# jasonyaw/CDAE

Hardware: AMD Instinct MI355X
Metric: users/sec (whole node) K=200 ML-10M-shape; Recall@10 parity (higher is better)
Workload: dtype f32

## Files before the change

cdae_amd/csrc/cdae_hip.hip:

```cpp
#include <hip/hip_runtime.h>

#include <cstring>

#include <rocprim/rocprim.hpp>

#include <algorithm>
#include <atomic>
#include <condition_variable>
#include <deque>
#include <mutex>
#include <thread>
#include <chrono>
#include <cmath>
#include <cstdarg>
#include <cstdlib>
#include <cstdio>
#include <cstring>
#include <numeric>
#include <string>
#include <vector>

#include "../../include/cdae_hip.h"
#include "cdae_internal.hpp"
#include "cdae_kernels.hpp"
// ... 1364 lines not shown
  place(CDAE_P_B, h->Kp); place(CDAE_P_B_AG, h->Kp);
  h->n_shared = o;
  CHK(dev_alloc(&h->d_shared, h->n_shared));
  HIPCHK(hipMemset(h->d_shared, 0, h->n_shared * sizeof(float)));
  const size_t WR = (size_t)h->wu_rows();
  h->cnt[CDAE_P_WU] = h->cnt[CDAE_P_WU_AG] = WR * h->Kp;
  CHK(dev_alloc(&h->d_Wu, WR * h->Kp));
  CHK(dev_alloc(&h->d_Wu_ag, WR * h->Kp));
  HIPCHK(hipMemset(h->d_Wu, 0, std::max<size_t>(WR * h->Kp, 1) * sizeof(float)));
  HIPCHK(hipMemset(h->d_Wu_ag, 0, std::max<size_t>(WR * h->Kp, 1) * sizeof(float)));
  if (h->cfg.linear_function) {
    h->cnt[CDAE_P_UU] = h->cnt[CDAE_P_UU_AG] = WR * h->Kp;
    CHK(dev_alloc(&h->d_Uu, WR * h->Kp));
    CHK(dev_alloc(&h->d_Uu_ag, WR * h->Kp));
  }

  const uint32_t B = (uint32_t)std::min<uint64_t>(h->B, U);
  uint64_t emax = 0;
  for (uint64_t s0 = 0; s0 < U; ++s0) {
    const uint64_t s1 = std::min<uint64_t>(U, s0 + B);
    emax = std::max<uint64_t>(emax, (uint64_t)(row_ptr[s1] - row_ptr[s0]));
  }
  h->ex_per_pos = h->mf == 2 ? 2u * h->hp.num_neg : 1u + h->hp.num_neg;
  h->Ecap = emax * h->ex_per_pos;
  h->h_grow_ptr.clear(); h->h_gunit_ptr.clear();
  if (h->shard_sampled()) {
    const int64_t* grp = h->g_row_ptr_src;
    const uint32_t* gcl = h->g_col_src;
    h->g_row_ptr_src = nullptr; h->g_col_src = nullptr;
    if (grp[0] != 0) return fail("whole-row row_ptr[0] must be 0");
    h->h_grow_ptr.assign(grp, grp + U + 1);
    uint64_t gmax = 0;
    for (uint64_t s0 = 0; s0 < U; ++s0) gmax = std::max<uint64_t>(gmax, (uint64_t)(grp[std::min<uint64_t>(U, s0 + B)] - grp[s0]));
    h->Ecap = gmax * h->ex_per_pos;
    const size_t gnnz = (size_t)grp[U];
    CHK(dev_alloc(&h->d_grow_ptr, U + 1)); CHK(dev_alloc(&h->d_gcol, gnnz));
    HIPCHK(hipMemcpy(h->d_grow_ptr, grp, (U + 1) * sizeof(int64_t), hipMemcpyHostToDevice));
    HIPCHK(hipMemcpy(h->d_gcol, gcl, gnnz * sizeof(uint32_t), hipMemcpyHostToDevice));
    h->h_gunit_ptr.assign(U + 1, 0u);
    for (uint64_t u = 0; u < U; ++u)
      h->h_gunit_ptr[u + 1] = h->h_gunit_ptr[u] + (uint32_t)((grp[u + 1] - grp[u] + h->hp.unit_pos - 1) / h->hp.unit_pos);
    CHK(dev_alloc(&h->d_gunit_ptr, U + 1));
    HIPCHK(hipMemcpy(h->d_gunit_ptr, h->h_gunit_ptr.data(), (U + 1) * sizeof(uint32_t), hipMemcpyHostToDevice));
    std::vector<uint32_t> guser(h->h_gunit_ptr[U]);
    for (uint64_t u = 0; u < U; ++u)
      for (uint32_t g = h->h_gunit_ptr[u]; g < h->h_gunit_ptr[u + 1]; ++g) guser[g] = (uint32_t)u;
    CHK(dev_alloc(&h->d_gunit_user, std::max<size_t>(guser.size(), 1)));
    HIPCHK(hipMemcpy(h->d_gunit_user, guser.data(), guser.size() * sizeof(uint32_t), hipMemcpyHostToDevice));
  }
  h->seq = 0; h->pre_n = 0;
  h->counting_sort = I <= cdae::TILE_SORT_MAX_ITEMS && DEV_ENV("CDAE_SORT_TILE") != nullptr;
  h->bucket_sort = false; h->bucket_ranges = 0; h->cell_units = 0;
  {
    const uint64_t BUCKET_MAX_EXAMPLES = h->cfg.full_output ? 100000 : 600000;
    const uint64_t keys = I + (h->shard_sampled() ? 1u : 0u);
    if (keys <= 65536 && !h->counting_sort && !h->mf_seq && h->Ecap <= BUCKET_MAX_EXAMPLES && h->Ecap > 0 && !DEV_ENV("CDAE_SORT_LIBRARY")) {
      const double b_share = (double)B / (double)U;
      const double draw_items = (double)(h->shard_sampled() ? h->I_global : I);
      const double whole_nnz = h->shard_sampled() ? (double)h->h_grow_ptr[U] : (double)nnz;
      const uint32_t negs = h->mf == 2 ? 2u * h->hp.num_neg - 0u : h->hp.num_neg;
      const double neg_per_item = b_share * whole_nnz * (double)negs / draw_items;
      std::vector<double> wgt(I);
      double total = 0.0;
      for (uint64_t i = 0; i < I; ++i) { wgt[i] = b_share * (double)pop[i] + neg_per_item; total += wgt[i]; }
      const double per_range = std::max(total / 256.0, std::min(2730.0, total / 8.0));
      std::vector<uint32_t> cut{0u};
      double acc = 0.0;
      for (uint64_t i = 0; i < I; ++i) {
        acc += wgt[i];
        if (i + 1 < I && (acc >= per_range || (i + 1) - cut.back() == cdae::BK_ITEMS)) { cut.push_back((uint32_t)(i + 1)); acc = 0.0; }
      }
      cut.push_back((uint32_t)I);
      if (cut.size() - 1 <= cdae::BK_MAX_RANGES) {
        h->bucket_sort = true;
        h->bucket_ranges = (uint32_t)cut.size() - 1;
        CHK(dev_alloc(&h->d_bucket_cut, cut.size()));
        HIPCHK(hipMemcpy(h->d_bucket_cut, cut.data(), cut.size() * sizeof(uint32_t), hipMemcpyHostToDevice));
        if (!h->mf && h->bucket_ranges <= cdae::BKC_MAX_RANGES && h->Ecap < (1ull << (32 - cdae::BKC_ITEM_BITS)) && !DEV_ENV("CDAE_SORT_SCAN")) {
          std::vector<uint16_t> rof(I);
          for (uint32_t r = 0; r + 1 < cut.size(); ++r)
            for (uint32_t i = cut[r]; i < cut[r + 1]; ++i) rof[i] = (uint16_t)r;
          CHK(dev_alloc(&h->d_range_of, (size_t)I));
          HIPCHK(hipMemcpy(h->d_range_of, rof.data(), I * sizeof(uint16_t), hipMemcpyHostToDevice));
        }
      }
    }
  }
  h->h_unit_ptr.assign(U + 1, 0u);
  for (uint64_t u = 0; u < U; ++u)
    h->h_unit_ptr[u + 1] = h->h_unit_ptr[u] + (uint32_t)((row_ptr[u + 1] - row_ptr[u] + h->hp.unit_pos - 1) / h->hp.unit_pos);
  h->unit_cap = 0;
  for (uint64_t s0 = 0; s0 < U; ++s0) {
    const uint64_t s1 = std::min<uint64_t>(U, s0 + B);
    h->unit_cap = std::max(h->unit_cap, h->h_unit_ptr[s1] - h->h_unit_ptr[s0]);
  }
  {
    std::vector<uint32_t> per(U);
    for (uint64_t u = 0; u < U; ++u) per[u] = h->h_unit_ptr[u + 1] - h->h_unit_ptr[u];
    std::partial_sort(per.begin(), per.begin() + B, per.end(), std::greater<uint32_t>());
    uint64_t top = 0;
    for (uint32_t i = 0; i < B; ++i) top += per[i];
    h->unit_cap = (uint32_t)std::max<uint64_t>(h->unit_cap, top);
  }
  if (h->shard_sampled())
    for (uint64_t s0 = 0; s0 < U; ++s0)
      h->unit_cap = std::max(h->unit_cap, h->h_gunit_ptr[std::min<uint64_t>(U, s0 + B)] - h->h_gunit_ptr[s0]);
  CHK(dev_alloc(&h->d_unit_ptr, U + 1));
// ... 1428 lines not shown
```

cdae_amd/csrc/cdae_kernels.hpp:

```cpp
#pragma once
#include <type_traits>

#include <hip/hip_runtime.h>
#include <stdint.h>

#include "../../include/cdae_rng.h"
#include "cdae_exchange_algebra.h"

namespace cdae {

constexpr int WAVE = 64;
constexpr uint32_t SLOT_MASK = 0x0FFFFFFFu;
constexpr uint32_t DUP_PREV_BIT = 1u << 28;
constexpr uint32_t DUP_NEXT_BIT = 1u << 29;
constexpr uint32_t DUP_NONE = 0xFFFFFFFFu;
constexpr uint32_t DUP_STRIPES = 64;
constexpr uint32_t TARGET_BIT = 1u << 30;
constexpr uint32_t INPUT_BIT = 1u << 31;

constexpr uint32_t LATE_MAX = 64;
struct DecodeLate {
  float* Ghot;
  uint32_t* hotdup;
  uint32_t late_rows;
// ... 134 lines not shown

__device__ __forceinline__ float loss_grad(uint32_t loss_type, float pred, float truth) {
  if (loss_type == 0u) return -2.f * (truth - pred);
  return fast_rcp(1.f + fast_exp(-pred)) - truth;
}
__device__ __forceinline__ float loss_eval(uint32_t loss_type, float pred, float truth) {
  if (loss_type == 0u) { float e = truth - pred; return e * e; }
  float ret = (1.f - truth) * pred;
  if (pred > 18.f) return ret + fast_exp(-pred);
  if (pred < -18.f) return ret - pred;
  return ret + log1pf(fast_exp(-pred));
}
__device__ __forceinline__ float activate(const HyperParams& hp, float x) {
  if (hp.linear) return x;
  if (!hp.tanh_act) return x > 18.f ? 1.f : (x < -18.f ? 0.f : fast_rcp(1.f + fast_exp(-x)));
  if (x > 9.f) return 1.f;
  if (x < -9.f) return -1.f;
  float r = fast_exp(-2.f * x);
  return (1.f - r) * fast_rcp(1.f + r);
}
__device__ __forceinline__ float act_deriv(const HyperParams& hp, float z) {
  return hp.linear ? 1.f : (hp.tanh_act ? 1.f - z * z : z - z * z);
}
template <bool ADA>
__device__ __forceinline__ void ada_step_t(const HyperParams& hp, float& p, float& acc, float grad) {
  if (ADA) {
    acc = fmaf(grad, grad, acc);
    p = fmaf(-hp.lr * grad, fast_rcp(fast_sqrt(acc) + hp.beta), p);
  } else {
    p = fmaf(-hp.lr, grad, p);
  }
}
__device__ __forceinline__ void ada_step(const HyperParams& hp, float& p, float& acc, float grad) {
  if (hp.adagrad) ada_step_t<true>(hp, p, acc, grad); else ada_step_t<false>(hp, p, acc, grad);
}

template <int CTRL, int ROW_MASK = 0xF>
__device__ __forceinline__ float dpp_add(float v) {
  const int moved = __builtin_amdgcn_update_dpp(0, __builtin_bit_cast(int, v), CTRL, ROW_MASK, 0xF,  true);
  return v + __builtin_bit_cast(float, moved);
}
__device__ __forceinline__ float wave_sum(float v) {
  v = dpp_add<0xB1>(v);
  v = dpp_add<0x4E>(v);
  v = dpp_add<0x141>(v);
  v = dpp_add<0x140>(v);
  v = dpp_add<0x142>(v);
  v = dpp_add<0x143>(v);
  return __builtin_bit_cast(float, __builtin_amdgcn_readlane(__builtin_bit_cast(int, v), 63));
}

constexpr uint32_t BKC_SLOTS = 32, BKC_ITEM_BITS = 12, BKC_ITEM_MASK = (1u << BKC_ITEM_BITS) - 1u;
constexpr uint32_t BKC_MAX_RANGES = 256;
constexpr uint32_t UNIT_POS_MAX = 128;

struct UnitRef { uint32_t slot, p0, p1; };

__device__ __forceinline__ UnitRef locate_unit(const uint32_t unit_pos, const uint32_t* __restrict__ uptr, uint32_t nb, uint32_t g,
                                               const uint32_t* __restrict__ unit_user = nullptr, uint64_t u0 = 0) {
  uint32_t lo = 0, hi = nb;
  if (unit_user) {
    lo = unit_user[g] - (uint32_t)u0;
  } else {
    while (hi - lo > 1) {
      const uint32_t mid = (lo + hi) >> 1;
      if (uptr[mid] <= g) lo = mid; else hi = mid;
    }
  }
  UnitRef r;
  r.slot = lo;
  r.p0 = (g - uptr[lo]) * unit_pos;
  r.p1 = r.p0 + unit_pos;
  return r;
}

__device__ __forceinline__ int lds_row_contains(const uint32_t* row, uint32_t n, uint32_t item) {
  uint32_t lo = 0, hi = n;
  while (lo < hi) {
    const uint32_t mid = (lo + hi) >> 1;
    if (row[mid] < item) lo = mid + 1; else hi = mid;
  }
  return lo < n && row[lo] == item;
}
constexpr uint32_t SAMPLE_LDS_ROW = 2048;

__global__ void __launch_bounds__(256)
sample_kernel(HyperParams hp, const int64_t* __restrict__ row_ptr, const uint32_t* __restrict__ col,
              const uint32_t* __restrict__ uptr, uint32_t n_units, uint64_t u0, uint32_t nb, uint32_t cidx,
              uint64_t seed, uint32_t epoch, uint32_t* __restrict__ ex_item, uint64_t* __restrict__ ex_val,
              uint16_t* __restrict__ ex_key16 ,
              uint32_t* __restrict__ seg , uint32_t seg_words,
              uint32_t* __restrict__ dup_count, uint32_t* __restrict__ dup_of_ex,
              const uint32_t* __restrict__ unit_user ,
              uint32_t* __restrict__ wg_state ,
              const uint32_t* __restrict__ gpos ,
              uint32_t shard_item0 = 0, uint32_t shard_items = 0, uint32_t draw_items = 0,
              const uint16_t* __restrict__ range_of = nullptr, const uint32_t* __restrict__ range_cut = nullptr, uint32_t n_ranges = 0,
              uint32_t* __restrict__ cells = nullptr, uint32_t* __restrict__ cell_flag = nullptr, uint32_t cell_tag = 0) {
#ifdef CDAE_PREP_SETPRIO
  __builtin_amdgcn_s_setprio(CDAE_PREP_SETPRIO);
#endif
  __shared__ uint32_t lds_rows[4][SAMPLE_LDS_ROW];
  __shared__ uint32_t cell_cnt[4][BKC_MAX_RANGES];
  __shared__ uint32_t cell_lo[BKC_MAX_RANGES];
  if (cells) {
    for (uint32_t i = threadIdx.x; i < n_ranges; i += blockDim.x) cell_lo[i] = range_cut[i];
// ... 1153 lines not shown
      if (dup) { const uint32_t k = len + (uint32_t)__popcll(dmask & below); lrow[k] = cur.di[h2] | DUP_ROW; lg[k] = 1.f; }
      if (mine) { const uint32_t k = len + n_d + (uint32_t)__popcll(mask & below); lrow[k] = cur.item[h2]; lg[k] = cur.g[h2]; }
      len += n_d + n_r;
    }
    __builtin_amdgcn_fence(__ATOMIC_RELEASE, "wavefront");
    __builtin_amdgcn_wave_barrier();
    const bool last = c0 + 2 * WAVE >= n_ex;
    while (len - head >= (uint32_t)TRIP) trip((uint32_t)TRIP);
    if (last || len + 4u * WAVE > GCAP) {
      if (len > head) trip(len - head);
      head = 0; len = 0;
      __builtin_amdgcn_wave_barrier();
    }
    cur = nxt;
  }
  if (lo >= hp.K) {
#pragma unroll
    for (int i = 0; i < NI; ++i) acc[i] = 0.f;
  }
  vstore<NI>(ga.HGpart + ((size_t)part * ga.n_units + unit) * hp.Kp + lo, acc);
  trace_end(hp, 5, unit * 8u + part, t0, n_ex);
}

template <int NI>
__global__ void __launch_bounds__(256)
hidden_gather_kernel(HyperParams hp, const int64_t* __restrict__ row_ptr, const uint32_t* __restrict__ uptr,
                     uint32_t n_units, uint64_t u0, uint32_t nb, const uint32_t* __restrict__ ex_item,
                     const float* __restrict__ G, const float* __restrict__ D0,
                     float* __restrict__ HGpart ,
                     uint32_t explicit_examples ,
                     const uint32_t* __restrict__ dup_of_ex, const float* __restrict__ dup_corr,
                     const uint32_t* __restrict__ unit_user,
                     const uint32_t* __restrict__ late_bits = nullptr ,
                     uint32_t late_words = 0) {
  __shared__ uint32_t gl_row[4][GATHER_CAP];
  __shared__ float gl_g[4][GATHER_CAP];
  __shared__ uint32_t lbits[LATE_BITS_WORDS];
  stage_late_bits(lbits, late_bits, late_words);
  const uint32_t part = blockIdx.x & 7u;
  const uint32_t unit = (blockIdx.x >> 3) * (blockDim.x / WAVE) + threadIdx.x / WAVE;
  if (unit >= n_units) return;
  const GatherArgs ga{row_ptr, uptr, n_units, u0, nb, ex_item, G, D0, HGpart, explicit_examples, dup_of_ex, dup_corr, unit_user,
                      late_bits, late_words, nullptr};
  hidden_gather_role<NI, false>(hp, ga, part, unit, gl_row[threadIdx.x / WAVE], gl_g[threadIdx.x / WAVE], late_bits ? lbits : nullptr);
}

struct FusedGeom {
  uint32_t hot_wgs;
  uint32_t decode_wgs;
  const uint32_t* cold_map;
};
constexpr uint32_t FUSED_LDS_WORDS = 4u * 2u * GATHER_CAP + LATE_BITS_WORDS;
static_assert(4u * ROWS16_LDS_WORDS <= FUSED_LDS_WORDS, "row roles' LDS");
static_assert(3u * (FUSED_LDS_WORDS + 8u) * 4u + 90376u <= 160u * 1024u, "three workgroups of this launch + one of bucket_sort_kernel per CU");
#ifndef CDAE_FUSED_WAVES_PER_SIMD
#define CDAE_FUSED_WAVES_PER_SIMD 3
#endif
template <int NV, int NT, int LOSS, bool ADAGRAD>
__global__ void __launch_bounds__(256, CDAE_FUSED_WAVES_PER_SIMD)
decode_gather_kernel(HyperParams hp, uint32_t hot_rows, FusedGeom geo, DecodeLate late, GatherArgs ga, CDAE_DECODE_PARAMS) {
  constexpr int CH = NT == 0 ? NV : NV + 1;
  constexpr int NI = CH <= 1 ? 1 : (CH <= 2 ? 2 : 4);
  __shared__ uint32_t fused_lds[FUSED_LDS_WORDS + 8u];
  const uint32_t wg = blockIdx.x;
  const uint32_t wid = __builtin_amdgcn_readfirstlane(threadIdx.x / WAVE);
  if (wg < geo.hot_wgs) {
    const uint32_t row = wg * 4u + wid;
    if (row < hot_rows && !CDAE_SKIP_ROLE(hp, 4u)) {
      const unsigned long long t0 = trace_begin(hp);
      __builtin_amdgcn_s_setprio(CDAE_HOT_PRIO);
      decode_row64<NI, LOSS, ADAGRAD, false, true>(hp, row, reinterpret_cast<float*>(fused_lds + wid * ROWS16_LDS_WORDS), ROW64_PARK_WORDS, late,
                                                   CDAE_DECODE_PASS);
      __builtin_amdgcn_s_setprio(0);
      trace_end(hp, 3, row, t0, hp.trace ? hw_place() : 0u);
    }
  } else if (wg < geo.decode_wgs) {
    if (CDAE_SKIP_ROLE(hp, 8u)) return;
    uint32_t* const claim = fused_lds + FUSED_LDS_WORDS;
    if (threadIdx.x < 4) claim[threadIdx.x] = 0u;
    __syncthreads();
    const uint32_t simd = (__builtin_amdgcn_s_getreg((1 << 11) | (4 << 6) | 4) ) & 3u;
    if (threadIdx.x % WAVE == 0) atomicCAS(&claim[simd], 0u, 1u + wid);
    __syncthreads();
    const uint32_t cs[4] = {claim[0], claim[1], claim[2], claim[3]};
    int mine = -1;
#pragma unroll
    for (int q = 0; q < 4; ++q) if (cs[q] == 1u + wid) mine = q;
    if (mine < 0) {
      uint32_t before = 0, cnt = 0;
#pragma unroll
      for (int q = 0; q < 4; ++q) if (cs[q] && cs[q] - 1u < wid) ++before;
      const uint32_t j = wid - before;
#pragma unroll
      for (int q = 0; q < 4; ++q) if (!cs[q]) { if (cnt == j) mine = q; ++cnt; }
    }
    const uint32_t g = geo.cold_map[wg * 4u + (uint32_t)mine];
    if (g == 0xFFFFFFFFu) return;
    const unsigned long long t0 = trace_begin(hp);
    decode_rows16<NV, NT, LOSS, ADAGRAD, true>(hp, hot_rows + g * 4u, fused_lds + wid * ROWS16_LDS_WORDS, CDAE_DECODE_PASS);
    trace_end(hp, 4, hot_rows / 4u + g, t0, hp.trace ? hw_place() : 0u);
  } else {
    uint32_t* const lbits = fused_lds + 4u * 2u * GATHER_CAP;
    stage_late_bits(lbits, ga.late_bits, ga.late_words);
    const uint32_t gw = wg - geo.decode_wgs;
    const uint32_t part = gw & 7u, unit = (gw >> 3) * 4u + wid;
    if (unit >= ga.n_units) return;
    hidden_gather_role<NI, true>(hp, ga, part, unit, fused_lds + wid * 2u * GATHER_CAP,
// ... 718 lines not shown
```

cdae_amd/csrc/cdae_sort_kernels.hpp:

```cpp
#pragma once
#include <hip/hip_runtime.h>
#include <stdint.h>

#include "cdae_kernels.hpp"

namespace cdae {

#ifndef CDAE_SEGSORT_THREADS
#define CDAE_SEGSORT_THREADS 256
#endif
constexpr uint32_t SEGSORT_THREADS = CDAE_SEGSORT_THREADS;
#ifndef CDAE_SEGSORT_ITEMS
#define CDAE_SEGSORT_ITEMS 8
#endif
constexpr uint32_t SEGSORT_ITEMS = CDAE_SEGSORT_ITEMS;
#ifndef CDAE_SEGSORT_WINDOW
#define CDAE_SEGSORT_WINDOW 3072
#endif
constexpr uint32_t SEGSORT_WINDOW = CDAE_SEGSORT_WINDOW;

constexpr uint32_t TILE_SORT_MAX_ITEMS = 32768;
#ifndef CDAE_TILE_EX
#define CDAE_TILE_EX 4096
#endif
// ... 141 lines not shown
      uint32_t rank = 0;
      if (in_lds) {
        const uint64_t v = raw[q];
        uint32_t r[8] = {0, 0, 0, 0, 0, 0, 0, 0};
        uint32_t j = a;
        for (; j + 8 <= b; j += 8) {
#pragma unroll
          for (int t = 0; t < 8; ++t) r[t] += raw[j + t] < v ? 1u : 0u;
        }
        for (; j < b; ++j) r[0] += raw[j] < v ? 1u : 0u;
        rank = ((r[0] + r[1]) + (r[2] + r[3])) + ((r[4] + r[5]) + (r[6] + r[7]));
        srt[a + rank] = v;
      } else {
        const uint64_t v = bucketed_val[p0 + q];
        for (uint32_t j = a; j < b; ++j) rank += bucketed_val[p0 + j] < v ? 1u : 0u;
        sorted_val[p0 + a + rank] = v;
      }
    }
    __syncthreads();
    uint32_t my_dups = 0;
    for (uint32_t q = threadIdx.x; q < n; q += blockDim.x) {
      const uint32_t k = item_of(k0, p0 + q);
      const uint32_t a = item_off[k] - p0, b = item_off[k + 1] - p0;
      uint64_t v = in_lds ? srt[q] : sorted_val[p0 + q];
      const uint32_t slot = (uint32_t)v & SLOT_MASK;
      uint32_t flags = 0;
      if (q > a && ((uint32_t)(in_lds ? srt[q - 1] : sorted_val[p0 + q - 1]) & SLOT_MASK) == slot) flags |= DUP_PREV_BIT;
      if (q + 1 < b && ((uint32_t)(in_lds ? srt[q + 1] : sorted_val[p0 + q + 1]) & SLOT_MASK) == slot) flags |= DUP_NEXT_BIT;
      if (in_lds || flags) sorted_val[p0 + q] = v | flags;
      if (flags & DUP_PREV_BIT) ++my_dups;
    }
    uint32_t off = my_dups ? atomicAdd(&blk_count, my_dups) : 0u;
    __syncthreads();
    if (threadIdx.x == 0) { blk_base = blk_count ? atomicAdd(dup_count + blockIdx.x % stripes, blk_count) : 0u; blk_count = 0u; }
    __syncthreads();
    if (my_dups) {
      off += blk_base;
      const uint32_t stripe_cap = dup_cap / stripes, stripe0 = (blockIdx.x % stripes) * stripe_cap;
      for (uint32_t q = threadIdx.x; q < n; q += blockDim.x) {
        const uint64_t v = sorted_val[p0 + q];
        if (!((uint32_t)v & DUP_PREV_BIT)) continue;
        const uint32_t idx = off < stripe_cap ? stripe0 + off : DUP_NONE;
        ++off;
        dup_of_pos[p0 + q] = idx;
        dup_of_ex[(uint32_t)(v >> 32)] = idx;
      }
    }
    __syncthreads();
    k0 = k1;
  }
}

constexpr uint32_t BK_THREADS = 512;
constexpr uint32_t BK_WINDOW = 4096;
constexpr uint32_t BK_ITEMS = 2048;
constexpr uint32_t BK_WAVE_LIST = BK_WINDOW / (BK_THREADS / 64);
constexpr uint32_t BK_SPIN_CAP = 1u << 21;
constexpr uint32_t BK_MAX_RANGES = 1024;
constexpr uint32_t BK_CELL_UNITS_MAX = 16384;
constexpr size_t BK_LDS_BYTES = (size_t)BK_WINDOW * 8 * 2 + (size_t)BK_WINDOW * 2 + (size_t)(BK_ITEMS + 1) * 4 * 2 + 64 * 4;
static_assert(BK_ITEMS <= 4 * BK_THREADS && BK_ITEMS <= (1u << BKC_ITEM_BITS), "bk_block_scan takes 4 counters per thread; a cell entry holds the item in BKC_ITEM_BITS bits");

__device__ __forceinline__ void bk_block_scan(uint32_t* v, uint32_t n, uint32_t* wave_tot) {
  const uint32_t t = threadIdx.x, lane = t % WAVE, wid = t / WAVE;
  uint32_t c[4], sum = 0;
#pragma unroll
  for (uint32_t j = 0; j < 4; ++j) { c[j] = 4u * t + j < n ? v[4u * t + j] : 0u; sum += c[j]; }
  uint32_t incl = sum;
#pragma unroll
  for (int off = 1; off < WAVE; off <<= 1) {
    const uint32_t o = __shfl_up(incl, off, WAVE);
    if ((int)lane >= off) incl += o;
  }
  if (lane == WAVE - 1) wave_tot[wid] = incl;
  __syncthreads();
  uint32_t before = 0;
  for (uint32_t w = 0; w < wid; ++w) before += wave_tot[w];
  uint32_t run = before + incl - sum;
#pragma unroll
  for (uint32_t j = 0; j < 4; ++j) { if (4u * t + j < n) v[4u * t + j] = run; run += c[j]; }
  if (t == BK_THREADS - 1) v[n] = run;
  __syncthreads();
}

constexpr uint32_t BK_UNROLL = 4;
template <typename F>
__device__ __forceinline__ void bk_scan_keys(const uint16_t* __restrict__ keys, uint32_t n_ex, F&& f) {
  const uint32_t n8 = n_ex & ~7u;
  constexpr uint32_t ROUND = BK_THREADS * 8u * BK_UNROLL;
  uint4 q[BK_UNROLL], nx[BK_UNROLL];
  auto request = [&](uint4 (&dst)[BK_UNROLL], uint32_t r0) {
#pragma unroll
    for (uint32_t u = 0; u < BK_UNROLL; ++u) {
      const uint32_t e0 = r0 + (u * BK_THREADS + threadIdx.x) * 8u;
      dst[u] = e0 < n8 ? *reinterpret_cast<const uint4*>(keys + e0) : make_uint4(0xFFFFFFFFu, 0xFFFFFFFFu, 0xFFFFFFFFu, 0xFFFFFFFFu);
    }
  };
  request(q, 0u);
  for (uint32_t r0 = 0; r0 < n8; r0 += ROUND) {
    const bool more = r0 + ROUND < n8;
    if (more) request(nx, r0 + ROUND);
#pragma unroll
    for (uint32_t u = 0; u < BK_UNROLL; ++u) {
      const uint32_t e0 = r0 + (u * BK_THREADS + threadIdx.x) * 8u;
      if (r0 + u * BK_THREADS * 8u >= n8) break;
      const bool valid = e0 < n8;
      const uint32_t w[4] = {q[u].x, q[u].y, q[u].z, q[u].w};
#pragma unroll
      for (uint32_t j = 0; j < 4; ++j) { f(e0 + 2u * j, w[j] & 0xFFFFu, valid); f(e0 + 2u * j + 1u, w[j] >> 16, valid); }
    }
    if (more) {
#pragma unroll
      for (uint32_t u = 0; u < BK_UNROLL; ++u) q[u] = nx[u];
    }
  }
  if (n_ex != n8 && threadIdx.x < WAVE) {
    const bool valid = threadIdx.x < n_ex - n8;
    f(n8 + threadIdx.x, valid ? (uint32_t)keys[n8 + threadIdx.x] : 0u, valid);
  }
}

__global__ void __launch_bounds__(BK_THREADS)
bucket_sort_kernel(const uint16_t* __restrict__ keys, const uint64_t* __restrict__ ex_val, uint32_t n_ex,
                   const uint32_t* __restrict__ range_cut , uint32_t* __restrict__ wg_state ,
                   const uint32_t* __restrict__ cells , uint32_t cell_units,
                   const uint32_t* __restrict__ cell_flag , uint32_t cell_tag,
                   uint32_t* __restrict__ seg_begin, uint32_t* __restrict__ seg_end, const uint32_t* __restrict__ rank_of,
                   uint32_t* __restrict__ segr_begin, uint32_t* __restrict__ segr_end, uint64_t* __restrict__ sorted_val,
                   uint64_t* __restrict__ scratch_val ,
                   uint32_t* __restrict__ dup_count, uint32_t dup_cap, uint32_t* __restrict__ dup_of_pos,
                   uint32_t* __restrict__ dup_of_ex , uint32_t stripes,
                   uint32_t* __restrict__ err ) {
#ifdef CDAE_PREP_SETPRIO
  __builtin_amdgcn_s_setprio(CDAE_PREP_SETPRIO);
#endif
  extern __shared__ __attribute__((aligned(16))) unsigned char bk_lds[];
  uint64_t* raw = reinterpret_cast<uint64_t*>(bk_lds);
  uint64_t* srt = raw + BK_WINDOW;
  uint32_t* off = reinterpret_cast<uint32_t*>(srt + BK_WINDOW);
  uint32_t* cur = off + BK_ITEMS + 1;
  uint32_t* misc = cur + BK_ITEMS + 1;
  uint16_t* raw_item = reinterpret_cast<uint16_t*>(misc + 64);
  const uint32_t t = threadIdx.x, w = blockIdx.x, lane = t % WAVE;
  const uint32_t lo = range_cut[w], n_it = range_cut[w + 1] - lo;
  for (uint32_t i = t; i <= n_it; i += BK_THREADS) off[i] = 0u;
  if (t == 0) { misc[16] = 0u; misc[17] = 0u; misc[19] = 0u; }
  __syncthreads();

  bool listed = false;
  bool scanned = false;
  if (cells && cell_units <= BK_CELL_UNITS_MAX && *cell_flag != cell_tag) {
    uint16_t* wcnt = reinterpret_cast<uint16_t*>(raw);
    uint32_t* lst = reinterpret_cast<uint32_t*>(srt);
    uint16_t* tk = reinterpret_cast<uint16_t*>(lst + BK_WINDOW);
    const uint32_t* mine = cells + (size_t)w * cell_units * BKC_SLOTS;
    const uint32_t per = (cell_units + BK_THREADS - 1) / BK_THREADS, u0 = min(cell_units, t * per), u1 = min(cell_units, u0 + per);
    uint32_t sum = 0;
    for (uint32_t u = u0; u < u1; ++u) { const uint32_t c = mine[(size_t)u * BKC_SLOTS]; wcnt[u] = (uint16_t)c; sum += c; }
    uint32_t incl = sum;
#pragma unroll
    for (int o = 1; o < WAVE; o <<= 1) {
      const uint32_t v = __shfl_up(incl, o, WAVE);
      if ((int)lane >= o) incl += v;
    }
    if (lane == WAVE - 1) misc[t / WAVE] = incl;
    __syncthreads();
    uint32_t pos = incl - sum, total = 0;
    for (uint32_t v = 0; v < BK_THREADS / WAVE; ++v) { if (v < t / WAVE) pos += misc[v]; total += misc[v]; }
    __syncthreads();
    if (total <= BK_WINDOW) {
      for (uint32_t u = u0; u < u1; ++u) {
        const uint32_t c = wcnt[u];
        for (uint32_t j = 0; j < c; ++j) lst[pos + j] = mine[(size_t)u * BKC_SLOTS + 1u + j];
        pos += c;
      }
      __syncthreads();
      for (uint32_t i = t; i < total; i += BK_THREADS) tk[i] = (uint16_t)atomicAdd(&off[lst[i] & BKC_ITEM_MASK], 1u);
      __syncthreads();
      bk_block_scan(off, n_it, misc);
      for (uint32_t i = t; i < total; i += BK_THREADS) {
        const uint32_t ent = lst[i], d = ent & BKC_ITEM_MASK, p = off[d] + tk[i];
        raw[p] = ex_val[ent >> BKC_ITEM_BITS];
        raw_item[p] = (uint16_t)d;
      }
      listed = true; scanned = true;
    } else {
      for (uint32_t i = t; i <= n_it; i += BK_THREADS) off[i] = 0u;
      __syncthreads();
    }
  }

  uint64_t* const wave_list = srt + (t / WAVE) * BK_WAVE_LIST;
  uint32_t wave_n = 0;
  if (!scanned) {
    bk_scan_keys(keys, n_ex, [&](uint32_t e, uint32_t k, bool valid) {
      const uint32_t d = k - lo;
      const bool mine = valid && d < n_it;
      const uint64_t m = __ballot(mine);
      if (m == 0ull) return;
      if (mine) {
        const uint32_t ticket = atomicAdd(&off[d], 1u);
        const uint32_t slot = wave_n + __builtin_amdgcn_mbcnt_hi((uint32_t)(m >> 32), __builtin_amdgcn_mbcnt_lo((uint32_t)m, 0u));
        if (slot < BK_WAVE_LIST) wave_list[slot] = ((uint64_t)e << 32) | (uint64_t)(d << 16) | (uint64_t)(ticket & 0xFFFFu);
      }
      wave_n += (uint32_t)__popcll(m);
    });
    if (wave_n > BK_WAVE_LIST && lane == 0) misc[19] = 1u;
    __syncthreads();
    bk_block_scan(off, n_it, misc);
  }

  if (t == 0) __hip_atomic_store(&wg_state[w], off[n_it] + 1u, __ATOMIC_RELEASE, __HIP_MEMORY_SCOPE_AGENT);
  for (uint32_t r = t; r < w; r += BK_THREADS) {
    uint32_t v, spin = 0;
    while ((v = __hip_atomic_load(&wg_state[r], __ATOMIC_ACQUIRE, __HIP_MEMORY_SCOPE_AGENT)) == 0u) {
      if (++spin > BK_SPIN_CAP) { v = 1u; __hip_atomic_store(err, 2u, __ATOMIC_RELAXED, __HIP_MEMORY_SCOPE_SYSTEM); break; }
      __builtin_amdgcn_s_sleep(1);
    }
    atomicAdd(&misc[16], v - 1u);
  }
  __syncthreads();
  const uint32_t base = misc[16];
  for (uint32_t i = t; i < n_it; i += BK_THREADS) {
    const uint32_t c = off[i + 1] - off[i], b = c ? base + off[i] : 0u, e = c ? base + off[i + 1] : 0u;
    seg_begin[lo + i] = b; seg_end[lo + i] = e;
    if (rank_of) { const uint32_t r = rank_of[lo + i]; segr_begin[r] = b; segr_end[r] = e; }
  }
  const bool wave_listed = !listed && misc[19] == 0u && off[n_it] <= BK_WINDOW;

  uint32_t ia = 0;
  while (ia < n_it) {
    uint32_t ib = ia + 1;
    {
      uint32_t l = ia + 1, h = n_it;
      while (l < h) { const uint32_t mid = (l + h + 1) >> 1; if (off[mid] - off[ia] <= BK_WINDOW) l = mid; else h = mid - 1; }
      ib = l;
    }
    const uint32_t g0 = off[ia], n = off[ib] - g0;
    const bool in_lds = n <= BK_WINDOW;
    if (n == 0) { ia = ib; continue; }
    if (listed) {
    } else if (wave_listed) {
      for (uint32_t i = lane; i < wave_n; i += WAVE) {
        const uint64_t rec = wave_list[i];
        const uint32_t d = (uint32_t)(rec >> 16) & 0xFFFFu, p = off[d] + ((uint32_t)rec & 0xFFFFu);
        raw[p] = ex_val[(uint32_t)(rec >> 32)];
        raw_item[p] = (uint16_t)d;
      }
    } else {
      for (uint32_t i = ia + t; i < ib; i += BK_THREADS) cur[i] = off[i] - g0;
      __syncthreads();
      bk_scan_keys(keys, n_ex, [&](uint32_t e, uint32_t k, bool valid) {
        const uint32_t d = k - lo;
        if (valid && d - ia < ib - ia) {
          const uint32_t p = atomicAdd(&cur[d], 1u);
          const uint64_t v = ex_val[e];
          if (in_lds) { raw[p] = v; raw_item[p] = (uint16_t)d; } else scratch_val[base + g0 + p] = v;
        }
      });
    }
    __threadfence_block();
    __syncthreads();
    for (uint32_t q = t; q < n; q += BK_THREADS) {
      if (in_lds) {
        const uint32_t d = raw_item[q], a = off[d] - g0, b = off[d + 1] - g0;
        const uint64_t v = raw[q];
        uint32_t r[8] = {0, 0, 0, 0, 0, 0, 0, 0};
        uint32_t j = a;
        for (; j + 8 <= b; j += 8) {
#pragma unroll
          for (int u = 0; u < 8; ++u) r[u] += raw[j + u] < v ? 1u : 0u;
        }
        for (; j < b; ++j) r[0] += raw[j] < v ? 1u : 0u;
        srt[a + ((r[0] + r[1]) + (r[2] + r[3])) + ((r[4] + r[5]) + (r[6] + r[7]))] = v;
      } else {
        const uint64_t v = scratch_val[base + g0 + q];
        uint32_t rank = 0;
        for (uint32_t j = 0; j < n; ++j) rank += scratch_val[base + g0 + j] < v ? 1u : 0u;
        sorted_val[base + g0 + rank] = v;
      }
    }
    __threadfence_block();
    __syncthreads();
    uint32_t my_dups = 0;
    for (uint32_t q = t; q < n; q += BK_THREADS) {
      uint32_t a = 0, b = n;
      if (in_lds) {
        uint32_t l = ia, h = ib - 1;
        while (l < h) { const uint32_t mid = (l + h + 1) >> 1; if (off[mid] - g0 <= q) l = mid; else h = mid - 1; }
        a = off[l] - g0; b = off[l + 1] - g0;
      }
      const uint64_t v = in_lds ? srt[q] : sorted_val[base + g0 + q];
      const uint32_t slot = (uint32_t)v & SLOT_MASK;
      uint32_t flags = 0;
      if (q > a && ((uint32_t)(in_lds ? srt[q - 1] : sorted_val[base + g0 + q - 1]) & SLOT_MASK) == slot) flags |= DUP_PREV_BIT;
      if (q + 1 < b && ((uint32_t)(in_lds ? srt[q + 1] : sorted_val[base + g0 + q + 1]) & SLOT_MASK) == slot) flags |= DUP_NEXT_BIT;
      if (in_lds || flags) sorted_val[base + g0 + q] = v | flags;
      if (flags & DUP_PREV_BIT) ++my_dups;
    }
    uint32_t o = my_dups ? atomicAdd(&misc[17], my_dups) : 0u;
    __syncthreads();
    if (t == 0) { misc[18] = misc[17] ? atomicAdd(dup_count + w % stripes, misc[17]) : 0u; misc[17] = 0u; }
    __syncthreads();
    if (my_dups) {
      o += misc[18];
      const uint32_t stripe_cap = dup_cap / stripes, stripe0 = (w % stripes) * stripe_cap;
      for (uint32_t q = t; q < n; q += BK_THREADS) {
        const uint64_t v = sorted_val[base + g0 + q];
        if (!((uint32_t)v & DUP_PREV_BIT)) continue;
        const uint32_t idx = o < stripe_cap ? stripe0 + o : DUP_NONE;
        ++o;
        dup_of_pos[base + g0 + q] = idx;
        dup_of_ex[(uint32_t)(v >> 32)] = idx;
      }
    }
    __syncthreads();
    ia = ib;
  }
}

}
```

Baseline: 2.913 million.

## Compact bucket sort LDS entries to 32-bit keys and read cells with vector loads

```diff
diff --git a/cdae_amd/csrc/cdae_hip.hip b/cdae_amd/csrc/cdae_hip.hip
--- a/cdae_amd/csrc/cdae_hip.hip
+++ b/cdae_amd/csrc/cdae_hip.hip
@@ -1440,7 +1440,10 @@
   h->counting_sort = I <= cdae::TILE_SORT_MAX_ITEMS && DEV_ENV("CDAE_SORT_TILE") != nullptr;
   h->bucket_sort = false; h->bucket_ranges = 0; h->cell_units = 0;
   {
-    const uint64_t BUCKET_MAX_EXAMPLES = h->cfg.full_output ? 100000 : 600000;
+    constexpr uint64_t BUCKET_MAX_EXAMPLES_FULL = 100000, BUCKET_MAX_EXAMPLES_SAMPLED = 600000;
+    static_assert(BUCKET_MAX_EXAMPLES_FULL < cdae::BK_MAX_EXAMPLES && BUCKET_MAX_EXAMPLES_SAMPLED < cdae::BK_MAX_EXAMPLES,
+                  "bucket_sort_kernel's LDS entries name an example in 32 - BKC_ITEM_BITS bits (cell path and scan fallback alike)");
+    const uint64_t BUCKET_MAX_EXAMPLES = h->cfg.full_output ? BUCKET_MAX_EXAMPLES_FULL : BUCKET_MAX_EXAMPLES_SAMPLED;
     const uint64_t keys = I + (h->shard_sampled() ? 1u : 0u);
     if (keys <= 65536 && !h->counting_sort && !h->mf_seq && h->Ecap <= BUCKET_MAX_EXAMPLES && h->Ecap > 0 && !DEV_ENV("CDAE_SORT_LIBRARY")) {
       const double b_share = (double)B / (double)U;
diff --git a/cdae_amd/csrc/cdae_kernels.hpp b/cdae_amd/csrc/cdae_kernels.hpp
--- a/cdae_amd/csrc/cdae_kernels.hpp
+++ b/cdae_amd/csrc/cdae_kernels.hpp
@@ -210,6 +210,9 @@
 
 constexpr uint32_t BKC_SLOTS = 32, BKC_ITEM_BITS = 12, BKC_ITEM_MASK = (1u << BKC_ITEM_BITS) - 1u;
 constexpr uint32_t BKC_MAX_RANGES = 256;
+constexpr uint32_t BK_WINDOW = 4096;
+constexpr uint32_t BK_ITEMS = 1024;
+constexpr uint32_t BK_LDS_BYTES = BK_WINDOW * 4u * 2u + (BK_ITEMS + 1u) * 4u * 2u + 64u * 4u;
 constexpr uint32_t UNIT_POS_MAX = 128;
 
 struct UnitRef { uint32_t slot, p0, p1; };
@@ -1469,7 +1472,8 @@
 };
 constexpr uint32_t FUSED_LDS_WORDS = 4u * 2u * GATHER_CAP + LATE_BITS_WORDS;
 static_assert(4u * ROWS16_LDS_WORDS <= FUSED_LDS_WORDS, "row roles' LDS");
-static_assert(3u * (FUSED_LDS_WORDS + 8u) * 4u + 90376u <= 160u * 1024u, "three workgroups of this launch + one of bucket_sort_kernel per CU");
+static_assert(3u * (FUSED_LDS_WORDS + 8u) * 4u + 2u * BK_LDS_BYTES <= 160u * 1024u, "three workgroups of this launch + two of bucket_sort_kernel per CU");
+static_assert(4u * (FUSED_LDS_WORDS + 8u) * 4u + BK_LDS_BYTES <= 160u * 1024u, "or four of this launch + one of bucket_sort_kernel");
 #ifndef CDAE_FUSED_WAVES_PER_SIMD
 #define CDAE_FUSED_WAVES_PER_SIMD 3
 #endif
diff --git a/cdae_amd/csrc/cdae_sort_kernels.hpp b/cdae_amd/csrc/cdae_sort_kernels.hpp
--- a/cdae_amd/csrc/cdae_sort_kernels.hpp
+++ b/cdae_amd/csrc/cdae_sort_kernels.hpp
@@ -217,14 +217,14 @@
 }
 
 constexpr uint32_t BK_THREADS = 512;
-constexpr uint32_t BK_WINDOW = 4096;
-constexpr uint32_t BK_ITEMS = 2048;
+constexpr uint32_t BK_PER = BK_WINDOW / BK_THREADS;
 constexpr uint32_t BK_WAVE_LIST = BK_WINDOW / (BK_THREADS / 64);
 constexpr uint32_t BK_SPIN_CAP = 1u << 21;
 constexpr uint32_t BK_MAX_RANGES = 1024;
 constexpr uint32_t BK_CELL_UNITS_MAX = 16384;
-constexpr size_t BK_LDS_BYTES = (size_t)BK_WINDOW * 8 * 2 + (size_t)BK_WINDOW * 2 + (size_t)(BK_ITEMS + 1) * 4 * 2 + 64 * 4;
+constexpr uint32_t BK_MAX_EXAMPLES = 1u << (32 - BKC_ITEM_BITS);
 static_assert(BK_ITEMS <= 4 * BK_THREADS && BK_ITEMS <= (1u << BKC_ITEM_BITS), "bk_block_scan takes 4 counters per thread; a cell entry holds the item in BKC_ITEM_BITS bits");
+static_assert(BK_WINDOW % BK_THREADS == 0 && BKC_SLOTS == 32, "a thread owns BK_PER sorted positions; eight lanes read one 128-byte cell");
 
 __device__ __forceinline__ void bk_block_scan(uint32_t* v, uint32_t n, uint32_t* wave_tot) {
   const uint32_t t = threadIdx.x, lane = t % WAVE, wid = t / WAVE;
@@ -286,7 +286,7 @@
 }
 
 __global__ void __launch_bounds__(BK_THREADS)
-bucket_sort_kernel(const uint16_t* __restrict__ keys, const uint64_t* __restrict__ ex_val, uint32_t n_ex,
+bucket_sort_kernel(const uint16_t* __restrict__ keys, const uint64_t* __restrict__ ex_val, uint32_t n_ex ,
                    const uint32_t* __restrict__ range_cut , uint32_t* __restrict__ wg_state ,
                    const uint32_t* __restrict__ cells , uint32_t cell_units,
                    const uint32_t* __restrict__ cell_flag , uint32_t cell_tag,
@@ -300,54 +300,61 @@
   __builtin_amdgcn_s_setprio(CDAE_PREP_SETPRIO);
 #endif
   extern __shared__ __attribute__((aligned(16))) unsigned char bk_lds[];
-  uint64_t* raw = reinterpret_cast<uint64_t*>(bk_lds);
-  uint64_t* srt = raw + BK_WINDOW;
-  uint32_t* off = reinterpret_cast<uint32_t*>(srt + BK_WINDOW);
+  uint32_t* plc = reinterpret_cast<uint32_t*>(bk_lds);
+  uint32_t* srt = plc + BK_WINDOW;
+  uint32_t* off = srt + BK_WINDOW;
   uint32_t* cur = off + BK_ITEMS + 1;
   uint32_t* misc = cur + BK_ITEMS + 1;
-  uint16_t* raw_item = reinterpret_cast<uint16_t*>(misc + 64);
   const uint32_t t = threadIdx.x, w = blockIdx.x, lane = t % WAVE;
   const uint32_t lo = range_cut[w], n_it = range_cut[w + 1] - lo;
   for (uint32_t i = t; i <= n_it; i += BK_THREADS) off[i] = 0u;
-  if (t == 0) { misc[16] = 0u; misc[17] = 0u; misc[19] = 0u; }
+  if (t == 0) { misc[16] = 0u; misc[17] = 0u; misc[19] = 0u; misc[20] = 0u; }
   __syncthreads();
 
   bool listed = false;
   bool scanned = false;
   if (cells && cell_units <= BK_CELL_UNITS_MAX && *cell_flag != cell_tag) {
-    uint16_t* wcnt = reinterpret_cast<uint16_t*>(raw);
-    uint32_t* lst = reinterpret_cast<uint32_t*>(srt);
-    uint16_t* tk = reinterpret_cast<uint16_t*>(lst + BK_WINDOW);
-    const uint32_t* mine = cells + (size_t)w * cell_units * BKC_SLOTS;
-    const uint32_t per = (cell_units + BK_THREADS - 1) / BK_THREADS, u0 = min(cell_units, t * per), u1 = min(cell_units, u0 + per);
-    uint32_t sum = 0;
-    for (uint32_t u = u0; u < u1; ++u) { const uint32_t c = mine[(size_t)u * BKC_SLOTS]; wcnt[u] = (uint16_t)c; sum += c; }
-    uint32_t incl = sum;
-#pragma unroll
-    for (int o = 1; o < WAVE; o <<= 1) {
-      const uint32_t v = __shfl_up(incl, o, WAVE);
-      if ((int)lane >= o) incl += v;
-    }
-    if (lane == WAVE - 1) misc[t / WAVE] = incl;
-    __syncthreads();
-    uint32_t pos = incl - sum, total = 0;
-    for (uint32_t v = 0; v < BK_THREADS / WAVE; ++v) { if (v < t / WAVE) pos += misc[v]; total += misc[v]; }
-    __syncthreads();
+    constexpr uint32_t BK_CELL_UNROLL = 4;
+    const uint4* mine = reinterpret_cast<const uint4*>(cells + (size_t)w * cell_units * BKC_SLOTS);
+    const uint32_t n4 = cell_units * (BKC_SLOTS / 4u);
+    for (uint32_t i0 = 0; i0 < n4; i0 += BK_THREADS * BK_CELL_UNROLL) {
+      uint4 c4[BK_CELL_UNROLL];
+#pragma unroll
+      for (uint32_t u = 0; u < BK_CELL_UNROLL; ++u) {
+        const uint32_t i = i0 + u * BK_THREADS + t;
+        c4[u] = i < n4 ? mine[i] : make_uint4(0u, 0u, 0u, 0u);
+      }
+#pragma unroll
+      for (uint32_t u = 0; u < BK_CELL_UNROLL; ++u) {
+        if (i0 + u * BK_THREADS >= n4) break;
+        const uint32_t cnt = __shfl(c4[u].x, (int)(lane & ~7u), WAVE);
+        const uint32_t s0 = 4u * (lane & 7u);
+        const uint32_t wd[4] = {c4[u].x, c4[u].y, c4[u].z, c4[u].w};
+        bool keep[4];
+        uint64_t m[4];
+        uint32_t tot = 0;
+#pragma unroll
+        for (uint32_t j = 0; j < 4; ++j) {
+          keep[j] = s0 + j >= 1u && s0 + j <= cnt;
+          m[j] = __ballot(keep[j]);
+          tot += (uint32_t)__popcll(m[j]);
+        }
+        if (tot == 0u) continue;
+        uint32_t at = 0;
+        if (lane == 0) at = atomicAdd(&misc[20], tot);
+        at = __shfl(at, 0, WAVE);
+#pragma unroll
+        for (uint32_t j = 0; j < 4; ++j) {
+          const uint32_t p = at + __builtin_amdgcn_mbcnt_hi((uint32_t)(m[j] >> 32), __builtin_amdgcn_mbcnt_lo((uint32_t)m[j], 0u));
+          if (keep[j] && p < BK_WINDOW) { srt[p] = wd[j]; atomicAdd(&off[wd[j] & BKC_ITEM_MASK], 1u); }
+          at += (uint32_t)__popcll(m[j]);
+        }
+      }
+    }
+    __syncthreads();
+    const uint32_t total = misc[20];
     if (total <= BK_WINDOW) {
-      for (uint32_t u = u0; u < u1; ++u) {
-        const uint32_t c = wcnt[u];
-        for (uint32_t j = 0; j < c; ++j) lst[pos + j] = mine[(size_t)u * BKC_SLOTS + 1u + j];
-        pos += c;
-      }
-      __syncthreads();
-      for (uint32_t i = t; i < total; i += BK_THREADS) tk[i] = (uint16_t)atomicAdd(&off[lst[i] & BKC_ITEM_MASK], 1u);
-      __syncthreads();
       bk_block_scan(off, n_it, misc);
-      for (uint32_t i = t; i < total; i += BK_THREADS) {
-        const uint32_t ent = lst[i], d = ent & BKC_ITEM_MASK, p = off[d] + tk[i];
-        raw[p] = ex_val[ent >> BKC_ITEM_BITS];
-        raw_item[p] = (uint16_t)d;
-      }
       listed = true; scanned = true;
     } else {
       for (uint32_t i = t; i <= n_it; i += BK_THREADS) off[i] = 0u;
@@ -355,7 +362,7 @@
     }
   }
 
-  uint64_t* const wave_list = srt + (t / WAVE) * BK_WAVE_LIST;
+  uint32_t* const wave_list = srt + (t / WAVE) * BK_WAVE_LIST;
   uint32_t wave_n = 0;
   if (!scanned) {
     bk_scan_keys(keys, n_ex, [&](uint32_t e, uint32_t k, bool valid) {
@@ -364,9 +371,9 @@
       const uint64_t m = __ballot(mine);
       if (m == 0ull) return;
       if (mine) {
-        const uint32_t ticket = atomicAdd(&off[d], 1u);
+        atomicAdd(&off[d], 1u);
         const uint32_t slot = wave_n + __builtin_amdgcn_mbcnt_hi((uint32_t)(m >> 32), __builtin_amdgcn_mbcnt_lo((uint32_t)m, 0u));
-        if (slot < BK_WAVE_LIST) wave_list[slot] = ((uint64_t)e << 32) | (uint64_t)(d << 16) | (uint64_t)(ticket & 0xFFFFu);
+        if (slot < BK_WAVE_LIST) wave_list[slot] = (e << BKC_ITEM_BITS) | d;
       }
       wave_n += (uint32_t)__popcll(m);
     });
@@ -375,10 +382,10 @@
     bk_block_scan(off, n_it, misc);
   }
 
-  if (t == 0) __hip_atomic_store(&wg_state[w], off[n_it] + 1u, __ATOMIC_RELEASE, __HIP_MEMORY_SCOPE_AGENT);
+  if (t == 0) __hip_atomic_store(&wg_state[w], off[n_it] + 1u, __ATOMIC_RELAXED, __HIP_MEMORY_SCOPE_AGENT);
   for (uint32_t r = t; r < w; r += BK_THREADS) {
     uint32_t v, spin = 0;
-    while ((v = __hip_atomic_load(&wg_state[r], __ATOMIC_ACQUIRE, __HIP_MEMORY_SCOPE_AGENT)) == 0u) {
+    while ((v = __hip_atomic_load(&wg_state[r], __ATOMIC_RELAXED, __HIP_MEMORY_SCOPE_AGENT)) == 0u) {
       if (++spin > BK_SPIN_CAP) { v = 1u; __hip_atomic_store(err, 2u, __ATOMIC_RELAXED, __HIP_MEMORY_SCOPE_SYSTEM); break; }
       __builtin_amdgcn_s_sleep(1);
     }
@@ -404,64 +411,80 @@
     const uint32_t g0 = off[ia], n = off[ib] - g0;
     const bool in_lds = n <= BK_WINDOW;
     if (n == 0) { ia = ib; continue; }
+    for (uint32_t i = ia + t; i < ib; i += BK_THREADS) cur[i] = off[i] - g0;
+    __syncthreads();
     if (listed) {
+      for (uint32_t i = t; i < n; i += BK_THREADS) { const uint32_t ent = srt[i]; plc[atomicAdd(&cur[ent & BKC_ITEM_MASK], 1u)] = ent; }
     } else if (wave_listed) {
-      for (uint32_t i = lane; i < wave_n; i += WAVE) {
-        const uint64_t rec = wave_list[i];
-        const uint32_t d = (uint32_t)(rec >> 16) & 0xFFFFu, p = off[d] + ((uint32_t)rec & 0xFFFFu);
-        raw[p] = ex_val[(uint32_t)(rec >> 32)];
-        raw_item[p] = (uint16_t)d;
-      }
+      for (uint32_t i = lane; i < wave_n; i += WAVE) { const uint32_t ent = wave_list[i]; plc[atomicAdd(&cur[ent & BKC_ITEM_MASK], 1u)] = ent; }
     } else {
-      for (uint32_t i = ia + t; i < ib; i += BK_THREADS) cur[i] = off[i] - g0;
-      __syncthreads();
       bk_scan_keys(keys, n_ex, [&](uint32_t e, uint32_t k, bool valid) {
         const uint32_t d = k - lo;
         if (valid && d - ia < ib - ia) {
           const uint32_t p = atomicAdd(&cur[d], 1u);
-          const uint64_t v = ex_val[e];
-          if (in_lds) { raw[p] = v; raw_item[p] = (uint16_t)d; } else scratch_val[base + g0 + p] = v;
+          if (in_lds) plc[p] = (e << BKC_ITEM_BITS) | d; else scratch_val[base + g0 + p] = ex_val[e];
         }
       });
     }
     __threadfence_block();
     __syncthreads();
-    for (uint32_t q = t; q < n; q += BK_THREADS) {
-      if (in_lds) {
-        const uint32_t d = raw_item[q], a = off[d] - g0, b = off[d + 1] - g0;
-        const uint64_t v = raw[q];
+    uint32_t my_dups = 0;
+    if (in_lds) {
+      for (uint32_t q = t; q < n; q += BK_THREADS) {
+        const uint32_t v = plc[q], d = v & BKC_ITEM_MASK, a = off[d] - g0, b = off[d + 1] - g0;
         uint32_t r[8] = {0, 0, 0, 0, 0, 0, 0, 0};
         uint32_t j = a;
         for (; j + 8 <= b; j += 8) {
 #pragma unroll
-          for (int u = 0; u < 8; ++u) r[u] += raw[j + u] < v ? 1u : 0u;
+          for (int u = 0; u < 8; ++u) r[u] += plc[j + u] < v ? 1u : 0u;
         }
-        for (; j < b; ++j) r[0] += raw[j] < v ? 1u : 0u;
+        for (; j < b; ++j) r[0] += plc[j] < v ? 1u : 0u;
         srt[a + ((r[0] + r[1]) + (r[2] + r[3])) + ((r[4] + r[5]) + (r[6] + r[7]))] = v;
-      } else {
+      }
+      __syncthreads();
+      uint64_t word[BK_PER];
+#pragma unroll
+      for (uint32_t k = 0; k < BK_PER; ++k) {
+        const uint32_t q = t + k * BK_THREADS;
+        word[k] = q < n ? ex_val[srt[q] >> BKC_ITEM_BITS] : 0ull;
+      }
+#pragma unroll
+      for (uint32_t k = 0; k < BK_PER; ++k) {
+        const uint32_t q = t + k * BK_THREADS;
+        if (q < n) plc[q] = (uint32_t)word[k];
+      }
+      __syncthreads();
+#pragma unroll
+      for (uint32_t k = 0; k < BK_PER; ++k) {
+        const uint32_t q = t + k * BK_THREADS;
+        if (q < n) {
+          const uint32_t d = srt[q] & BKC_ITEM_MASK, a = off[d] - g0, b = off[d + 1] - g0;
+          const uint32_t slot = (uint32_t)word[k] & SLOT_MASK;
+          uint32_t flags = 0;
+          if (q > a && (plc[q - 1] & SLOT_MASK) == slot) flags |= DUP_PREV_BIT;
+          if (q + 1 < b && (plc[q + 1] & SLOT_MASK) == slot) flags |= DUP_NEXT_BIT;
+          sorted_val[base + g0 + q] = word[k] | flags;
+          if (flags & DUP_PREV_BIT) ++my_dups;
+        }
+      }
+    } else {
+      for (uint32_t q = t; q < n; q += BK_THREADS) {
         const uint64_t v = scratch_val[base + g0 + q];
         uint32_t rank = 0;
         for (uint32_t j = 0; j < n; ++j) rank += scratch_val[base + g0 + j] < v ? 1u : 0u;
         sorted_val[base + g0 + rank] = v;
       }
-    }
-    __threadfence_block();
-    __syncthreads();
-    uint32_t my_dups = 0;
-    for (uint32_t q = t; q < n; q += BK_THREADS) {
-      uint32_t a = 0, b = n;
-      if (in_lds) {
-        uint32_t l = ia, h = ib - 1;
-        while (l < h) { const uint32_t mid = (l + h + 1) >> 1; if (off[mid] - g0 <= q) l = mid; else h = mid - 1; }
-        a = off[l] - g0; b = off[l + 1] - g0;
-      }
-      const uint64_t v = in_lds ? srt[q] : sorted_val[base + g0 + q];
-      const uint32_t slot = (uint32_t)v & SLOT_MASK;
-      uint32_t flags = 0;
-      if (q > a && ((uint32_t)(in_lds ? srt[q - 1] : sorted_val[base + g0 + q - 1]) & SLOT_MASK) == slot) flags |= DUP_PREV_BIT;
-      if (q + 1 < b && ((uint32_t)(in_lds ? srt[q + 1] : sorted_val[base + g0 + q + 1]) & SLOT_MASK) == slot) flags |= DUP_NEXT_BIT;
-      if (in_lds || flags) sorted_val[base + g0 + q] = v | flags;
-      if (flags & DUP_PREV_BIT) ++my_dups;
+      __threadfence_block();
+      __syncthreads();
+      for (uint32_t q = t; q < n; q += BK_THREADS) {
+        const uint64_t v = sorted_val[base + g0 + q];
+        const uint32_t slot = (uint32_t)v & SLOT_MASK;
+        uint32_t flags = 0;
+        if (q > 0 && ((uint32_t)sorted_val[base + g0 + q - 1] & SLOT_MASK) == slot) flags |= DUP_PREV_BIT;
+        if (q + 1 < n && ((uint32_t)sorted_val[base + g0 + q + 1] & SLOT_MASK) == slot) flags |= DUP_NEXT_BIT;
+        if (flags) sorted_val[base + g0 + q] = v | flags;
+        if (flags & DUP_PREV_BIT) ++my_dups;
+      }
     }
     uint32_t o = my_dups ? atomicAdd(&misc[17], my_dups) : 0u;
     __syncthreads();
```

Result: faster. 2.954 million (median of 6 runs) (+1.4%).
